# andrewkwolek/dynamic-visual-slam

Measured on AMD Instinct MI355X. Metric: frames/sec ORB+match @1280x720x2000kp, higher is better.
Workload: dtype u8

## Files before the change

### dynamic-visual-slam_amd/csrc/orb.hip

```cpp
#include <math.h>
#include <stdlib.h>
#include <string.h>
#include <algorithm>
#include <new>
#include <chrono>
#include <vector>
#include "common.h"
#include "cv_round.h"
#include "device_mem.h"
#ifdef DVS_TEST_HOOKS
#include "../../include/dvslam_hip_test.h"
#endif
#include "orb_kernels.h"

namespace dvs {

void launch_cand_mask(const Geom* d_geom, const Cell* d_cells, const CandMask& mk, uint32_t* cand, int* cellCount, int nimg, int c0, int c1,
                      hipStream_t st);

static inline short sat_short(int v) { return (short)(v < -32768 ? -32768 : (v > 32767 ? 32767 : v)); }
static inline uint64_t align_up(uint64_t v, uint64_t a) { return (v + a - 1) / a * a; }

}

// ... 43 lines not shown
  DeviceBuf<int> d_nodeof, d_celloff, d_candtotal;
  DeviceBuf<dvs_keypoint> d_kps;
  DeviceBuf<u8> d_desc;
  DeviceBuf<int> d_nout;
  PinnedBuf<dvs_keypoint> h_kps;
  PinnedBuf<u8> h_desc;
  PinnedBuf<int> h_nout;
  DeviceBuf<u8> d_mask;
  size_t octree_smem = 0;
  int octree_nmax = 0, octree_ptscap = 0;
  int oct_ncls = 0;
  int oct_l0[4] = {0, 0, 0, 0};
  size_t oct_smem_cls[3] = {0, 0, 0};
  int oct_nmax_cls[3] = {0, 0, 0}, oct_ptscap_cls[3] = {0, 0, 0};

  dvs_status ready(PyrSlot& s) { return s.pyr.get() ? DVS_OK : s.pyr.alloc(batch * geom.frameBytes + 256); }
  dvs_status ready(BlurSlot& s) { return s.blur.get() ? DVS_OK : s.blur.alloc(batch * geom.frameBytes); }
  dvs_status ready(CandSlot& s) {
    if (s.cellcount.get()) return DVS_OK;
    if (!s.done) DVS_HIP(s.done.create());
    DVS_TRY(s.cand.alloc(batch * geom.candPerFrame));
    return s.cellcount.alloc(batch * geom.totalCells);
  }
  dvs_status ready(LvlSlot& s) {
    if (s.lvlkp.get()) return DVS_OK;
    DVS_TRY(s.lvlcount.alloc(batch * geom.nlevels));
    return s.lvlkp.alloc(batch * (size_t)geom.kpBlock);
  }
  template <class Slot> dvs_status turn(Ring<Slot>& r) { r.advance(); return ready(r.cur()); }
  void rewind(int depth) { blur.rewind(depth); cand.rewind(depth); lvl.rewind(depth); pyr.depth = depth; }
};

enum {
  kEvFork,
  kEvBlur,
  kEvStart,
  kEvChainGate,
  kEvOct,
  kEvEnd,
  kEvPrefetch,
  kEvCount = kEvPrefetch + 2
};

struct dvs_orb {
  dvs_orb_params prm;
  int device = 0;
  hipStream_t own_stream = nullptr, stream = nullptr;
  hipStream_t pf_stream = nullptr;
  hipStream_t aux_stream = nullptr;
  Event ev[kEvCount];
  int pf_idx = 0;
  Event ev_level[DVS_MAX_LEVELS];
  bool overlap = true;
  bool single_stream = false;
  int max_batch = 1;
  std::vector<float> scale, inv_scale, sigma2, inv_sigma2;
  std::vector<int> feat_per_level;
  int umax[16];
  int rows = 0, cols = 0;
  Workspace ws;
  int ring = 3;
  int async_run = 0;
  Ring<Event> ev_outs;
  int out_gen = 0;
  bool out_pending = false;
  bool defer_outputs = false;
  hipEvent_t output_event = nullptr;
  hipEvent_t guard_event = nullptr;
  hipEvent_t after_fast_event = nullptr;
  hipEvent_t gate_event = nullptr;
  bool pf_joined = false;
  const u8* next_hint = nullptr;
  struct ChainGraph { const u8* img0; uint64_t step0, fstride0; int nimg; u8* pyr; hipGraph_t graph; hipGraphExec_t exec; };
  std::vector<ChainGraph> chain_graphs;
  int env_chain_graph = -1;
  int64_t chain_graph_launches = 0;
  bool pf_valid = false;
  const u8* pf_img = nullptr; uint64_t pf_step = 0, pf_fstride = 0; int pf_nimg = 0;
  int env_cascade = -1;
  int fast_byte_dma = 0;
  int env_blur_mfma = 0;
  int env_oct_threads = 0;
  int env_host_poll = 1;
  int env_desc_order = 1;
  PinnedBuf<int> h_seq;
  DeviceBuf<int> d_ticket;
  int export_seq = 0;
  bool async_oct = false, last_async = false;
  hipStream_t tail_stream = nullptr;
  CandMask mask{};
  int last_nimg = 0;
  ImgSrc last_src{};
  StageTimer timer;
};

namespace {

void drop_chain_graphs(dvs_orb* h) {
  for (auto& c : h->chain_graphs) {
    if (c.exec) (void)hipGraphExecDestroy(c.exec);
    if (c.graph) (void)hipGraphDestroy(c.graph);
  }
  h->chain_graphs.clear();
}

void free_workspace(dvs_orb* h) {
  h->ws = Workspace{};
  drop_chain_graphs(h);
  h->rows = h->cols = 0;
  h->out_gen = 0; h->pf_valid = false; h->next_hint = nullptr;
}

dvs_status quiesce(dvs_orb* h) {
  DVS_HIP(hipStreamSynchronize(h->stream));
  if (h->aux_stream) DVS_HIP(hipStreamSynchronize(h->aux_stream));
  if (h->pf_stream) DVS_HIP(hipStreamSynchronize(h->pf_stream));
  if (h->out_pending) DVS_HIP(hipEventSynchronize(h->ev_outs.cur()));
  h->out_pending = false;
  return DVS_OK;
}

void build_ctor_tables(dvs_orb* h) {
  const int nl = h->prm.nlevels;
  const double scaleFactor = (double)h->prm.scale_factor;
  h->scale.assign(nl, 0.f); h->sigma2.assign(nl, 0.f); h->inv_scale.assign(nl, 0.f); h->inv_sigma2.assign(nl, 0.f);
  h->scale[0] = 1.0f; h->sigma2[0] = 1.0f;
  for (int i = 1; i < nl; i++) {
    h->scale[i] = (float)(h->scale[i - 1] * scaleFactor);
    h->sigma2[i] = h->scale[i] * h->scale[i];
  }
  for (int i = 0; i < nl; i++) { h->inv_scale[i] = 1.0f / h->scale[i]; h->inv_sigma2[i] = 1.0f / h->sigma2[i]; }
  h->feat_per_level.assign(nl, 0);
  const float factor = (float)(1.0f / scaleFactor);
  float desired = h->prm.nfeatures * (1 - factor) / (1 - (float)pow((double)factor, (double)nl));
  int sum = 0;
  for (int l = 0; l < nl - 1; l++) {
    h->feat_per_level[l] = cv_round_f(desired);
    sum += h->feat_per_level[l];
    desired *= factor;
  }
  h->feat_per_level[nl - 1] = std::max(h->prm.nfeatures - sum, 0);
  int v, v0;
  const int vmax = cv_floor_f(kHalfPatch * sqrtf(2.f) / 2 + 1);
  const int vmin = cv_ceil_f(kHalfPatch * sqrtf(2.f) / 2);
  const double hp2 = kHalfPatch * kHalfPatch;
  for (v = 0; v <= vmax; ++v) h->umax[v] = cv_round_d(sqrt(hp2 - v * v));
  for (v = kHalfPatch, v0 = 0; v >= vmin; --v) {
    while (h->umax[v0] == h->umax[v0 + 1]) ++v0;
    h->umax[v] = v0;
    ++v0;
  }
}

void level_size(const dvs_orb* h, int rows, int cols, int level, int& lr, int& lc) {
  const float s = h->inv_scale[level];
  lc = cv_round_f((float)cols * s);
  lr = cv_round_f((float)rows * s);
}

void build_axis_table(int ssize, int dsize, bool clamp_like_x, std::vector<int>& ofs, std::vector<int>& coef) {
  const double inv_scale = (double)dsize / ssize;
  const double scale = 1. / inv_scale;
  for (int d = 0; d < dsize; d++) {
    float fx = (float)((d + 0.5) * scale - 0.5);
    int sx = cv_floor_f(fx);
    fx -= sx;
// ... 582 lines not shown

  if (h->overlap) {
    if (h->guard_event && !will_defer) { DVS_HIP(hipStreamWaitEvent(h->aux_stream, h->guard_event, 0)); h->guard_event = nullptr; }
    if (h->pf_valid && !sharded && !(h->defer_outputs && h->output_event)) { DVS_HIP(hipStreamWaitEvent(h->aux_stream, h->ev[kEvPrefetch + h->pf_idx], 0)); h->pf_joined = true; }
  }

  const bool tail = async && h->tail_stream != nullptr;
  if (tail) {
    h->timer.begin(DVS_STAGE_BLUR, st);
    launch_blur(h, src, nimg, st, cascade);
    h->timer.end(st);
  }

  if (ov) {
    int tail = G.nlevels;
    while (tail > 2 && G.lv[tail - 1].nCells * 16 < G.totalCells) tail--;
    for (int l = 0; l <= tail && l < G.nlevels; l++) {
      const int lastl = l == tail ? G.nlevels - 1 : l;
      if (lastl > 0) DVS_HIP(hipStreamWaitEvent(st, h->ev_level[lastl], 0));
      h->timer.begin(DVS_STAGE_FAST, st, l == 0);
      launch_fast(h, src, nimg, st, G.lv[l].cellBase, G.lv[lastl].cellBase + G.lv[lastl].nCells);
      h->timer.end(st);
    }
  } else {
    h->timer.begin(DVS_STAGE_FAST, st);
    if (sharded) {
      for (int l = 0; l < G.nlevels; l++)
        if ((src.levelMask >> l) & 1u) launch_fast(h, src, nimg, st, G.lv[l].cellBase, G.lv[l].cellBase + G.lv[l].nCells);
    } else {
      launch_fast(h, src, nimg, st, 0, G.totalCells);
    }
    h->timer.end(st);
  }
  hipStream_t bst = h->overlap ? h->aux_stream : st;
  hipEvent_t ev_fastdone = h->after_fast_event ? h->after_fast_event : h->ev[kEvFork];
  if (h->after_fast_event || h->overlap) DVS_HIP(hipEventRecord(ev_fastdone, st));

  if (pend) {
    DVS_TRY(W.turn(W.lvl));
  }
  hipStream_t qs = async ? bst : st;
  if (async) DVS_HIP(hipStreamWaitEvent(bst, ev_fastdone, 0));
  const int blurRows = (G.blurStrips + kOctTMax / 64 - 1) / (kOctTMax / 64);
  const bool fuse_blur = h->single_stream && !async && !sharded && !(h->env_blur_mfma && W.blur_mfma_ok) &&
                         blur_stream_ok(h, src, cascade) && (long)nimg * (G.nlevels + blurRows) <= 256;
  h->timer.begin(DVS_STAGE_OCTREE, qs);
  if (fuse_blur) {
    if (h->guard_event) { DVS_HIP(hipStreamWaitEvent(qs, h->guard_event, 0)); h->guard_event = nullptr; }
    hipLaunchKernelGGL(k_octree_blur, dim3(nimg, G.nlevels + blurRows), dim3(kOctTMax), W.octree_smem, qs, W.d_geom.get(), W.cand.cur().cand.get(), W.cand.cur().cellcount.get(),
                       W.d_celloff.get(), W.d_pts.get(), W.d_nodeof.get(), W.d_candtotal.get(), W.lvl.cur().lvlkp.get(), W.lvl.cur().lvlcount.get(), W.octree_nmax, W.octree_ptscap, src.levelMask,
                       G.nlevels, W.d_strips.get(), G.blurStrips, src, W.blur.cur().blur.get());
  } else {
    launch_octree(h, nimg, qs, src.levelMask, async && G.nlevels * nimg > 256);
  }
  h->timer.end(qs);
  if (async) { DVS_HIP(hipEventRecord(W.cand.cur().done, qs)); W.cand.cur().done_valid = true; }

  if (async) {}
  else if (bst != st) DVS_HIP(hipStreamWaitEvent(bst, ev_fastdone, 0));
  else if (h->guard_event) DVS_HIP(hipStreamWaitEvent(st, h->guard_event, 0));
  hipEvent_t late_guard = bst != st ? h->guard_event : nullptr;
  h->guard_event = nullptr;
  if (!tail && !fuse_blur) {
    h->timer.begin(DVS_STAGE_BLUR, bst);
    launch_blur(h, src, nimg, bst, cascade);
    h->timer.end(bst);
  }

  hipStream_t dst = st;
  if (will_defer) {
    dst = tail ? h->tail_stream : bst;
    if (tail) {
      DVS_HIP(hipStreamWaitEvent(dst, W.cand.cur().done, 0));
    } else if (!async) {
      DVS_HIP(hipEventRecord(h->ev[kEvOct], st));
      DVS_HIP(hipStreamWaitEvent(bst, h->ev[kEvOct], 0));
    }
    if (late_guard) DVS_HIP(hipStreamWaitEvent(dst, late_guard, 0));
  } else if (bst != st) {
    DVS_HIP(hipEventRecord(h->ev[kEvBlur], bst));
    DVS_HIP(hipStreamWaitEvent(st, h->ev[kEvBlur], 0));
  }
  h->timer.begin(DVS_STAGE_DESCRIBE, dst);
  if (h->env_desc_order && nimg >= 16) {
    hipLaunchKernelGGL(k_kp_order, dim3(nimg, G.nlevels), dim3(256), 0, dst, W.d_geom.get(), W.lvl.cur().lvlkp.get(), W.lvl.cur().lvlcount.get(), W.d_kpsorted.get(), W.d_kpsortidx.get());
    hipLaunchKernelGGL(k_describe, dim3((G.kpBlock + 4 * kDescKP - 1) / (4 * kDescKP), nimg), dim3(256), 0, dst, W.d_geom.get(), src, W.blur.cur().blur.get(),
                       W.d_kpsorted.get(), W.d_kpsortidx.get(), W.lvl.cur().lvlcount.get(), d_kps, d_desc, d_nout, capacity);
  } else {
    hipLaunchKernelGGL(k_describe, dim3((G.kpBlock + 4 * kDescKP - 1) / (4 * kDescKP), nimg), dim3(256), 0, dst, W.d_geom.get(), src, W.blur.cur().blur.get(),
                       W.lvl.cur().lvlkp.get(), W.d_kpident.get(), W.lvl.cur().lvlcount.get(), d_kps, d_desc, d_nout, capacity);
  }
  h->timer.end(dst);
  if (will_defer) {
    h->ev_outs.advance();
    h->out_gen++;
    DVS_HIP(hipEventRecord(h->ev_outs.cur(), dst));
    DVS_HIP(hipEventRecord(h->output_event, dst));
    h->out_pending = true;
    h->gate_event = nullptr;
  } else {
    h->gate_event = (may_defer && h->output_event) ? h->output_event : h->ev[kEvEnd];
    DVS_HIP(hipEventRecord(h->gate_event, st));
  }
  DVS_HIP(hipGetLastError());
  h->last_nimg = nimg;
  h->last_src = src;
  return DVS_OK;
}

}

extern "C" {

static dvs_status orb_create(const dvs_orb_params* params, int32_t device, bool single_stream, bool on_stream, hipStream_t ext, dvs_orb** out);
dvs_status dvs_orb_create(const dvs_orb_params* params, int32_t device, dvs_orb** out) { return orb_create(params, device, false, false, nullptr, out); }
DVS_HOOK dvs_status dvs_orb_create_single_stream(const dvs_orb_params* params, int32_t device, dvs_orb** out) { return orb_create(params, device, true, false, nullptr, out); }
DVS_HOOK dvs_status dvs_orb_create_on_stream(const dvs_orb_params* params, int32_t device, void* hip_stream, dvs_orb** out) {
  return orb_create(params, device, true, true, (hipStream_t)hip_stream, out);
}

static dvs_status orb_create(const dvs_orb_params* params, int32_t device, bool single_stream, bool on_stream, hipStream_t ext, dvs_orb** out) {
  DVS_ARG(params && out);
  *out = nullptr;
  DVS_ARG(params->nlevels >= 1 && params->nlevels <= DVS_MAX_LEVELS);
  DVS_ARG(params->nfeatures >= 0 && params->scale_factor > 1.0f && params->max_batch >= 0);
  DVS_TRY(check_device(device));
  dvs_orb* h = new (std::nothrow) dvs_orb();
  if (!h) { set_error("out of host memory"); return DVS_ERR_HIP; }
  h->prm = *params;
  bool allzero = true;
  for (int i = 0; i < 7; i++) allzero = allzero && params->gauss_kernel[i] == 0;
  if (allzero) { const int k[7] = {18, 34, 48, 56, 48, 34, 18}; memcpy(h->prm.gauss_kernel, k, sizeof(k)); }
  int ksum = 0;
  for (int i = 0; i < 7; i++) {
    ksum += h->prm.gauss_kernel[i];
    if (h->prm.gauss_kernel[i] < 0 || h->prm.gauss_kernel[i] > 255) ksum = 1 << 20;
  }
  if (ksum > 257) { delete h; set_error("gauss_kernel sum %d would overflow the Q8.8 row buffer", ksum); return DVS_ERR_ARG; }
  h->device = device;
  h->max_batch = params->max_batch > 0 ? params->max_batch : 1;
  if (on_stream) {
    h->stream = ext;
  } else {
    hipError_t e = hipStreamCreateWithFlags(&h->own_stream, hipStreamNonBlocking);
    if (e != hipSuccess) { delete h; set_error("hipStreamCreate: %s", hipGetErrorString(e)); return DVS_ERR_HIP; }
    h->stream = h->own_stream;
  }
  h->single_stream = single_stream;
  h->overlap = env_int("DVS_NO_OVERLAP", 0) == 0 && !single_stream;
  h->env_cascade = env_int("DVS_CASCADE", -1);
  h->env_chain_graph = env_int("DVS_CHAIN_GRAPH", -1);
  h->env_blur_mfma = env_int("DVS_BLUR_MFMA", 0);
  h->env_host_poll = env_int("DVS_HOST_POLL", 1);
  h->env_oct_threads = env_int("DVS_OCT_T", 0);
  h->env_desc_order = env_int("DVS_DESC_ORDER", 1);
  if (h->env_oct_threads != 0 && h->env_oct_threads != kOctT && h->env_oct_threads != kOctTMax) h->env_oct_threads = 0;
  h->fast_byte_dma = probe_byte_dma(device, h->stream) && env_int("DVS_FAST_BYTE_DMA", 1);
  int prio_lo = 0, prio_hi = 0;
  (void)hipDeviceGetStreamPriorityRange(&prio_lo, &prio_hi);
  bool ok = single_stream || (hipStreamCreateWithPriority(&h->aux_stream, hipStreamNonBlocking, prio_lo) == hipSuccess &&
                              hipStreamCreateWithPriority(&h->pf_stream, hipStreamNonBlocking, prio_hi) == hipSuccess);
  for (Event& e : h->ev) ok = ok && e.create() == hipSuccess;
  for (Event& e : h->ev_outs.slot) ok = ok && e.create() == hipSuccess;
  for (int l = 1; l < params->nlevels; l++) ok = ok && h->ev_level[l].create() == hipSuccess;
  h->ev_outs.rewind(h->ring - 1);
  if (!ok) {
    dvs_orb_destroy(h);
    set_error("stream / event creation failed");
    return DVS_ERR_HIP;
  }
  build_ctor_tables(h);
  *out = h;
  return DVS_OK;
}

void dvs_orb_destroy(dvs_orb* h) {
  if (!h) return;
  (void)hipSetDevice(h->device);
  (void)quiesce(h);
  h->timer.resolve();
  free_workspace(h);
  if (h->aux_stream) (void)hipStreamDestroy(h->aux_stream);
  if (h->pf_stream) (void)hipStreamDestroy(h->pf_stream);
  if (h->own_stream) (void)hipStreamDestroy(h->own_stream);
  delete h;
}

int32_t dvs_orb_max_keypoints(const dvs_orb* h) { return h ? h->prm.nfeatures + 3 * h->prm.nlevels : 0; }

dvs_status dvs_orb_set_stream(dvs_orb* h, void* s) {
  DVS_ARG(h);
  DVS_HIP(hipSetDevice(h->device));
  DVS_HIP(hipStreamSynchronize(h->stream));
  h->stream = (hipStream_t)s;
  return DVS_OK;
}
DVS_HOOK dvs_status dvs_orb_set_overlap(dvs_orb* h, int32_t on) {
  DVS_ARG(h);
  DVS_HIP(hipSetDevice(h->device));
  if (on && h->single_stream) { set_error("dvs_orb_set_overlap: this extractor was created with one stream only"); return DVS_ERR_UNSUPPORTED; }
  DVS_TRY(quiesce(h));
  h->pf_valid = false; h->pf_joined = false;
  h->overlap = on != 0;
  return DVS_OK;
}
DVS_HOOK dvs_status dvs_orb_set_async_quadtree(dvs_orb* h, int32_t on) {
  DVS_ARG(h);
  if (on && h->single_stream) { set_error("dvs_orb_set_async_quadtree: this extractor was created with one stream only"); return DVS_ERR_UNSUPPORTED; }
  DVS_HIP(hipSetDevice(h->device));
  DVS_TRY(quiesce(h));
  h->last_async = false;
  h->async_oct = on != 0;
  return DVS_OK;
}
DVS_HOOK int64_t dvs_orb_chain_graph_launches(const dvs_orb* h) { return h ? h->chain_graph_launches : 0; }

DVS_HOOK dvs_status dvs_orb_set_tail_stream(dvs_orb* h, void* hip_stream) {
  DVS_ARG(h);
  DVS_HIP(hipSetDevice(h->device));
  DVS_TRY(quiesce(h));
  h->tail_stream = (hipStream_t)hip_stream;
  h->ring = hip_stream ? 4 : 3;
  h->ws.rewind(h->ring); h->ev_outs.rewind(h->ring - 1); h->out_gen = 0; h->async_run = 0;
  for (CandSlot& c : h->ws.cand.slot) c.done_valid = false;
  h->last_async = false;
  return DVS_OK;
}
DVS_HOOK dvs_status dvs_orb_use_own_stream(dvs_orb* h) {
  DVS_ARG(h);
  if (!h->own_stream) { set_error("dvs_orb_use_own_stream: this extractor was created on a caller's stream and has none of its own"); return DVS_ERR_UNSUPPORTED; }
  DVS_HIP(hipSetDevice(h->device));
  DVS_HIP(hipStreamSynchronize(h->stream));
  h->stream = h->own_stream;
  return DVS_OK;
}
void* dvs_orb_get_stream(dvs_orb* h) { return h ? (void*)h->stream : nullptr; }

dvs_status dvs_orb_synchronize(dvs_orb* h) {
// ... 336 lines not shown
```

### dynamic-visual-slam_amd/csrc/orb_kernels.h

```cpp
#pragma once
#include <hip/hip_runtime.h>
#include "glibc_sincosf.h"
#include "lsort.h"
#include "orb_geom.h"
#include "orb_device_common.h"

namespace dvs {

typedef uint8_t u8;

struct ImgSrc {
  const u8* img0;
  uint64_t step0;
  uint64_t fstride0;
  u8* pyr;
  uint32_t levelMask;
  int32_t slotted;
};

__device__ __forceinline__ const u8* level_ptr(const Geom* g, const ImgSrc& s, int f, int l, int& pitch) {
  if (l == 0) { pitch = (int)s.step0; return s.img0 + (uint64_t)f * s.fstride0; }
  pitch = g->lv[l].pitch;
  return s.pyr + (uint64_t)f * g->frameBytes + g->lv[l].off;
}
// ... 1562 lines not shown
  if (!((src.levelMask >> it.level) & 1u)) return;
  const int lane = lane_id(), m = lane & 31, half = lane >> 5;
  const LevelGeom& L = g->lv[it.level];
  int pitch;
  const u8* img = level_ptr(g, src, f, it.level, pitch);
  u8* dst = blur + (uint64_t)f * g->frameBytes + L.off;
  const int W = L.w, H = L.h, dp = L.pitch;
  const int c0 = it.strip * 128 + 32 * wv;
  if (c0 >= W) return;
  const int ti = (it.tab + wv) * 2;
  const bv4i Bh1 = __builtin_bit_cast(bv4i, tab[(ti + 0) * 64 + lane]), Bh2 = __builtin_bit_cast(bv4i, tab[(ti + 1) * 64 + lane]);
  const bv4i Av0 = __builtin_bit_cast(bv4i, tab[(avt * 2 + 0) * 64 + lane]), Av1 = __builtin_bit_cast(bv4i, tab[(avt * 2 + 1) * 64 + lane]);
  const bv4i bias = {(int)0x80808080u, (int)0x80808080u, (int)0x80808080u, (int)0x80808080u};
  const bv16i zero = {0, 0, 0, 0, 0, 0, 0, 0, 0, 0, 0, 0, 0, 0, 0, 0};
  constexpr uint32_t kC = 65536u + (32768u << 8);
  const uint32_t col1 = (uint32_t)min(max(c0 - 16 + 16 * half, 0), pitch - 16), col2 = (uint32_t)min(max(c0 + 16 + 16 * half, 0), pitch - 16);
  auto row_off = [&](int vr) -> uint32_t {
    int r = vr < 0 ? -vr : vr;
    r = r >= H ? 2 * H - 2 - r : r;
    r = min(max(r, 0), H - 1);
    return (uint32_t)r * (uint32_t)pitch;
  };
  bv4i r1, r2;
  auto issue = [&](int b) {
    const uint32_t ro = row_off(32 * b - 3 + m);
    r1 = *reinterpret_cast<const bv4i*>(img + ro + col1);
    r2 = *reinterpret_cast<const bv4i*>(img + ro + col2);
  };
  auto hcomp = [&](const bv4i& x1, const bv4i& x2, bv4i& hi, bv4i& lo) {
    bv16i acc = __builtin_amdgcn_mfma_i32_32x32x32_i8(x1 ^ bias, Bh1, zero, 0, 0, 0);
    acc = __builtin_amdgcn_mfma_i32_32x32x32_i8(x2 ^ bias, Bh2, acc, 0, 0, 0);
    uint32_t P[8];
#pragma unroll
    for (int q = 0; q < 8; q++) P[q] = __builtin_amdgcn_perm((uint32_t)acc[2 * q + 1], (uint32_t)acc[2 * q], 0x05040100u);
#pragma unroll
    for (int d = 0; d < 4; d++) {
      hi[d] = (int)__builtin_amdgcn_perm(P[2 * d + 1], P[2 * d], 0x07050301u);
      lo[d] = (int)(__builtin_amdgcn_perm(P[2 * d + 1], P[2 * d], 0x06040200u) ^ 0x80808080u);
    }
  };
  const int ocol = c0 + 16 * half;
  uint32_t so = (uint32_t)(32 * it.t0 + m) * (uint32_t)dp + (uint32_t)ocol;
  auto vtile = [&](int t, const bv4i& chi, const bv4i& clo, const bv4i& nhi, const bv4i& nlo) {
    bv16i lo = __builtin_amdgcn_mfma_i32_32x32x32_i8(clo, Av0, zero, 0, 0, 0);
    lo = __builtin_amdgcn_mfma_i32_32x32x32_i8(nlo, Av1, lo, 0, 0, 0);
#pragma unroll
    for (int k = 0; k < 16; k++) lo[k] = (int)(((uint32_t)lo[k] + kC) >> 8);
    bv16i u = __builtin_amdgcn_mfma_i32_32x32x32_i8(chi, Av0, lo, 0, 0, 0);
    u = __builtin_amdgcn_mfma_i32_32x32x32_i8(nhi, Av1, u, 0, 0, 0);
    uint32_t o[4];
#pragma unroll
    for (int d = 0; d < 4; d++) {
      const uint32_t p01 = __builtin_amdgcn_perm((uint32_t)u[4 * d + 1], (uint32_t)u[4 * d], 0x0c0c0501u);
      const uint32_t p23 = __builtin_amdgcn_perm((uint32_t)u[4 * d + 3], (uint32_t)u[4 * d + 2], 0x0c0c0501u);
      o[d] = p01 | (p23 << 16);
    }
    const auto s02 = __builtin_amdgcn_permlane32_swap(o[0], o[2], false, false);
    const auto s13 = __builtin_amdgcn_permlane32_swap(o[1], o[3], false, false);
    if (32 * t + m < H && ocol < W) *reinterpret_cast<uint4*>(dst + so) = make_uint4(s02[0], s02[1], s13[0], s13[1]);
    so += 32u * (uint32_t)dp;
  };
  bv4i hiA, loA, hiB, loB;
  issue(it.t0);
  bv4i x1 = r1, x2 = r2;
  issue(it.t0 + 1);
  hcomp(x1, x2, hiA, loA);
  const int tend = it.t0 + it.nt;
  for (int t = it.t0; t < tend; t += 2) {
    x1 = r1; x2 = r2;
    if (t + 1 < tend) issue(t + 2);
    hcomp(x1, x2, hiB, loB);
    vtile(t, hiA, loA, hiB, loB);
    if (t + 1 < tend) {
      x1 = r1; x2 = r2;
      if (t + 2 < tend) issue(t + 3);
      hcomp(x1, x2, hiA, loA);
      vtile(t + 1, hiB, loB, hiA, loA);
    }
  }
}

constexpr int kDescKP = 8;
constexpr int kWinR = 18, kWinRows = 2 * kWinR + 1, kWinPitch = 48;
__global__ __launch_bounds__(256) void k_kp_order(const Geom* __restrict__ g, const uint32_t* __restrict__ lvlKp, const int* __restrict__ lvlKpCount,
                                                  uint32_t* __restrict__ sortedKp, uint32_t* __restrict__ sortedIdx) {
  __shared__ uint32_t key[kMaxQuota + 8];
  const int f = blockIdx.x, level = blockIdx.y;
  const LevelGeom& L = g->lv[level];
  const int n = min(lvlKpCount[f * g->nlevels + level], min(L.N + 4, kMaxQuota + 8));
  const uint32_t* in = lvlKp + (uint64_t)f * g->kpBlock + L.kpOff;
  uint32_t* outK = sortedKp + (uint64_t)f * g->kpBlock + L.kpOff;
  uint32_t* outI = sortedIdx + (uint64_t)f * g->kpBlock + L.kpOff;
  for (int i = threadIdx.x; i < n; i += 256) {
    const uint32_t pk = in[i];
    key[i] = ((uint32_t)(pt_y(pk) >> 5) << 20) | ((uint32_t)(pt_x(pk) >> 7) << 12) | (uint32_t)i;
  }
  __syncthreads();
  for (int i = threadIdx.x; i < n; i += 256) {
    const uint32_t k = key[i];
    int rank = 0;
    for (int j = 0; j < n; j++) rank += key[j] < k ? 1 : 0;
    outK[rank] = in[i];
    outI[rank] = (uint32_t)i;
  }
}

__global__ __launch_bounds__(256) void k_describe(const Geom* __restrict__ g, ImgSrc src, const u8* __restrict__ blur,
                                                  const uint32_t* __restrict__ lvlKp, const uint32_t* __restrict__ lvlKpIdx, const int* __restrict__ lvlKpCount,
                                                  dvs_keypoint* __restrict__ outKp, u8* __restrict__ outDesc,
                                                  int* __restrict__ nOut, int capacity) {
  typedef uint4 __attribute__((aligned(1))) uint4u;
  __shared__ __attribute__((aligned(16))) u8 win[4][2][kWinRows * kWinPitch];
  DVS_CHAIN_PRIO();
  const int wg = xcd_contiguous_id();
  const int f = wg / (int)gridDim.x, bx = wg - f * (int)gridDim.x;
  const int lane = lane_id();
  const int wv = __builtin_amdgcn_readfirstlane(threadIdx.x >> 6);
  const int nl = g->nlevels;
  const int* cnt = lvlKpCount + f * nl;
  const int slot0 = (bx * 4 + wv) * kDescKP;
  if (bx == 0 && threadIdx.x == 0) {
    if (src.slotted) {
      for (int l = 0; l < nl; l++) nOut[f * nl + l] = cnt[l];
    } else {
      int total = 0;
      for (int l = 0; l < nl; l++) total += cnt[l];
      nOut[f] = min(total, capacity);
    }
  }
  if (slot0 >= g->kpBlock) return;
  const int slot = min(slot0 + (lane & 7), g->kpBlock - 1);
  const uint32_t pkRaw = lvlKp[(uint64_t)f * g->kpBlock + slot];
  const uint32_t idxRaw = lvlKpIdx[(uint64_t)f * g->kpBlock + slot];
  int level = 0, pre = 0, acc = 0;
  for (int l = 0; l < nl; l++) {
    if (slot >= g->lv[l].kpOff) { level = l; pre = acc; }
    acc += cnt[l];
  }
  const LevelGeom& L = g->lv[level];
  const bool inlist = slot - L.kpOff < cnt[level];
  const int idx = inlist ? (int)idxRaw : slot - L.kpOff;
  const int gi = src.slotted ? L.kpOff + idx : pre + idx;
  const bool valid = slot0 + (lane & 7) < g->kpBlock && inlist && gi < capacity;
  if ((__ballot(valid) & 0xffull) == 0) return;
  const uint32_t pk = valid ? pkRaw : 0u;
  const int lvl = valid ? level : 0;
  const int x = pt_x(pk) + kMinBorder + (valid ? 0 : 3), y = pt_y(pk) + kMinBorder + (valid ? 0 : 3);
  const uint64_t pyrOff = (uint64_t)f * g->frameBytes + g->lv[lvl].off;
  const u8* imgL = lvl == 0 ? src.img0 + (uint64_t)f * src.fstride0 : src.pyr + pyrOff;
  const int pitchL = lvl == 0 ? (int)src.step0 : g->lv[lvl].pitch;
  const u8* blurL = blur + pyrOff;
  const int bpL = g->lv[lvl].pitch;
#define DVS_RL(v, i) __builtin_amdgcn_readlane((int)(v), (i))
#define DVS_RLP(p, i) reinterpret_cast<const u8*>(((uint64_t)(uint32_t)DVS_RL((uint32_t)((uint64_t)(p) >> 32), i) << 32) | (uint32_t)DVS_RL((uint32_t)(uint64_t)(p), i))
  const int prow = min(lane >> 1, 2 * kHalfPatch), half = lane & 1;
  const int v = prow - kHalfPatch;
  const int pcol = half ? 1 : -kHalfPatch;
  uint4 d[kDescKP];
#pragma unroll
  for (int i = 0; i < kDescKP; i++) {
    const u8* ib = DVS_RLP(imgL, i);
    const int pi = DVS_RL(pitchL, i), xi = DVS_RL(x, i), yi = DVS_RL(y, i);
    d[i] = *reinterpret_cast<const uint4u*>(ib + (uint32_t)(mul_i24(yi + v, pi) + xi + pcol));
  }
  const int e0 = lane, e1 = 64 + lane;
  const int wr0 = e0 / 3, wc0 = e0 - 3 * wr0, wr1 = min(e1 / 3, kWinRows - 1), wc1 = e1 - 3 * (e1 / 3);
  const bool w1ok = e1 < kWinRows * 3;
  static_assert(kDescKP == 8, "the window registers below are named per keypoint");
  uint4 wq0_0, wq0_1, wq0_2, wq0_3, wq0_4, wq0_5, wq0_6, wq0_7, wq1_0, wq1_1, wq1_2, wq1_3, wq1_4, wq1_5, wq1_6, wq1_7;
#define DVS_REQUEST_WINDOW(i)                                                                                  \
  {                                                                                                            \
    const u8* bb = DVS_RLP(blurL, i);                                                                          \
    const int bp = DVS_RL(bpL, i), xi = DVS_RL(x, i), yi = DVS_RL(y, i);                                       \
    const int xa = (xi - kWinR) & ~3;   \
    const u8* o = bb + (int64_t)(yi - kWinR) * bp + xa;                                                        \
    wq0_##i = *reinterpret_cast<const uint4*>(o + (uint32_t)(mul_i24(wr0, bp) + 16 * wc0));                    \
    wq1_##i = *reinterpret_cast<const uint4*>(o + (uint32_t)(mul_i24(wr1, bp) + 16 * wc1));                    \
  }
  DVS_REQUEST_WINDOW(0) DVS_REQUEST_WINDOW(1) DVS_REQUEST_WINDOW(2) DVS_REQUEST_WINDOW(3)
  float px0[4], py0[4], px1[4], py1[4];
#pragma unroll
  for (int r = 0; r < 4; r++) {
    const int pat = reinterpret_cast<const int*>(c_pattern)[64 * r + lane];
    px0[r] = (float)(int8_t)(pat & 0xff); py0[r] = (float)(int8_t)((pat >> 8) & 0xff);
    px1[r] = (float)(int8_t)((pat >> 16) & 0xff); py1[r] = (float)(int8_t)((pat >> 24) & 0xff);
  }
  const uint32_t* wt = g->icw[lane];
  const uint32_t w0 = wt[0], w1 = wt[1], w2 = wt[2], w3 = wt[3], w4 = wt[4], w5 = wt[5], w6 = wt[6], w7 = wt[7];
  int q[2 * kDescKP];
#pragma unroll
  for (int i = 0; i < kDescKP; i++) {
    uint32_t su = __builtin_amdgcn_udot4(d[i].x, w0, 0u, false);
    su = __builtin_amdgcn_udot4(d[i].y, w1, su, false);
    su = __builtin_amdgcn_udot4(d[i].z, w2, su, false);
    su = __builtin_amdgcn_udot4(d[i].w, w3, su, false);
    uint32_t sm = __builtin_amdgcn_udot4(d[i].x, w4, 0u, false);
    sm = __builtin_amdgcn_udot4(d[i].y, w5, sm, false);
    sm = __builtin_amdgcn_udot4(d[i].z, w6, sm, false);
    sm = __builtin_amdgcn_udot4(d[i].w, w7, sm, false);
    q[i] = (int)su - kHalfPatch * (int)sm;
    q[kDescKP + i] = v * (int)sm;
  }
  DVS_REQUEST_WINDOW(4) DVS_REQUEST_WINDOW(5) DVS_REQUEST_WINDOW(6) DVS_REQUEST_WINDOW(7)
#define DVS_BFLY(n, o)                                        \
  {                                                           \
    const bool hi = (lane & (o)) != 0;                        \
    _Pragma("unroll") for (int j = 0; j < (n); j++) {         \
      const int keep = hi ? q[(n) + j] : q[j];                \
      const int send = hi ? q[j] : q[(n) + j];                \
      q[j] = keep + __shfl_xor(send, (o));                    \
    }                                                         \
  }
  DVS_BFLY(8, 32) DVS_BFLY(4, 16) DVS_BFLY(2, 8) DVS_BFLY(1, 4)
#undef DVS_BFLY
  int tot = q[0];
  tot += __shfl_xor(tot, 2);
  tot += __shfl_xor(tot, 1);
  const int other = __shfl_xor(tot, 32);
  const int m10 = lane < 32 ? tot : other, m01 = lane < 32 ? other : tot;
  const float angleK = fast_atan2_deg((float)m01, (float)m10);
  const float factorPI = (float)(3.14159265358979323846 / 180.f);
  const float arad = __fmul_rn(angleK, factorPI);
  const float cosK = gsc::cosf_(arad), sinK = gsc::sinf_(arad);
  const unsigned vmask = (unsigned)(__ballot(valid) & 0xffull);
  constexpr int kCsLane = 4;
  const int giL = gi;
  auto brief = [&](const int i, const uint4& wa, const uint4& wb) __attribute__((always_inline)) {
    u8* wl = win[wv][i & 1];
    *reinterpret_cast<uint4*>(wl + wr0 * kWinPitch + 16 * wc0) = wa;
    if (w1ok) *reinterpret_cast<uint4*>(wl + wr1 * kWinPitch + 16 * wc1) = wb;
    const int xi = DVS_RL(x, i);
    const int wxi = xi - ((xi - kWinR) & ~3);
    wave_lds_fence();
    const float a = __builtin_bit_cast(float, DVS_RL(__builtin_bit_cast(int, cosK), kCsLane * i));
    const float b = __builtin_bit_cast(float, DVS_RL(__builtin_bit_cast(int, sinK), kCsLane * i));
    const int bco = kWinR * kWinPitch + wxi - 32 * kWinPitch - 0x4B000020;
    unsigned long long words[4];
    typedef float f32x2 __attribute__((ext_vector_type(2)));
    const f32x2 a2 = {a, a}, b2 = {b, b};
#pragma unroll
    for (int r = 0; r < 4; r++) {
      constexpr float kRound = 8388640.0f;
      const f32x2 kR2 = {kRound, kRound};
      const f32x2 pxv = {px0[r], px1[r]}, pyv = {py0[r], py1[r]};
      const f32x2 rowv = (pxv * b2 + pyv * a2) + kR2;
      const f32x2 colv = (pxv * a2 - pyv * b2) + kR2;
      const float fr0 = rowv[0], fr1 = rowv[1], fc0 = colv[0], fc1 = colv[1];
      const int r0 = __builtin_bit_cast(int, fr0), r1 = __builtin_bit_cast(int, fr1);
      const int c0 = __builtin_bit_cast(int, fc0), c1 = __builtin_bit_cast(int, fc1);
      const int t0 = wl[mad_i24(r0, kWinPitch, c0) + bco];
      const int t1 = wl[mad_i24(r1, kWinPitch, c1) + bco];
      words[r] = __ballot(t0 < t1);
    }
    if ((vmask >> i) & 1u) {
      const int gii = DVS_RL(giL, i);
      if (lane < 4) {
        const unsigned long long w = lane == 0 ? words[0] : lane == 1 ? words[1] : lane == 2 ? words[2] : words[3];
        reinterpret_cast<unsigned long long*>(outDesc + ((uint64_t)f * capacity + gii) * 32)[lane] = w;
      }
    }
  };
  brief(0, wq0_0, wq1_0); brief(1, wq0_1, wq1_1); brief(2, wq0_2, wq1_2); brief(3, wq0_3, wq1_3);
  brief(4, wq0_4, wq1_4); brief(5, wq0_5, wq1_5); brief(6, wq0_6, wq1_6); brief(7, wq0_7, wq1_7);
  const float angle = __shfl(angleK, kCsLane * (lane & 7));
  if (lane < kDescKP && valid) {
    dvs_keypoint kp;
    kp.x = (float)x; kp.y = (float)y;
    if (level != 0) { kp.x = __fmul_rn(kp.x, L.scale); kp.y = __fmul_rn(kp.y, L.scale); }
    kp.size = L.kpSize;
    kp.angle = angle;
    kp.response = (float)pt_s(pk);
    kp.octave = level;
    kp.class_id = -1;
    outKp[(uint64_t)f * capacity + gi] = kp;
  }
#undef DVS_REQUEST_WINDOW
#undef DVS_RL
#undef DVS_RLP
}

struct LevelBlockLayout { uint64_t blockBytes, kpsOff, descOff; int nl, kpBlock; int kpOff[DVS_MAX_LEVELS]; int owner[DVS_MAX_LEVELS]; };

__global__ __launch_bounds__(256) void k_merge_levels(LevelBlockLayout Y, const u8* __restrict__ blocks, int nimg, dvs_keypoint* __restrict__ outKp,
                                                      u8* __restrict__ outDesc, int capacity, int* __restrict__ nOut) {
  const int f = blockIdx.y;
  const int slot = blockIdx.x * 256 + threadIdx.x;
  int level = 0, pre = 0, acc = 0, cntL = 0;
  for (int l = 0; l < Y.nl; l++) {
    const int c = reinterpret_cast<const int*>(blocks + (uint64_t)Y.owner[l] * Y.blockBytes)[f * Y.nl + l];
    if (slot >= Y.kpOff[l]) { level = l; pre = acc; cntL = c; }
    acc += c;
  }
  if (slot == 0) nOut[f] = min(acc, capacity);
  if (slot >= Y.kpBlock) return;
  const int idx = slot - Y.kpOff[level], gi = pre + idx;
  if (idx >= cntL || gi >= capacity) return;
  const u8* blk = blocks + (uint64_t)Y.owner[level] * Y.blockBytes;
  const uint32_t* sk = reinterpret_cast<const uint32_t*>(blk + Y.kpsOff) + ((uint64_t)f * Y.kpBlock + slot) * 7;
  uint32_t* dk = reinterpret_cast<uint32_t*>(outKp) + ((uint64_t)f * capacity + gi) * 7;
#pragma unroll
  for (int k = 0; k < 7; k++) dk[k] = sk[k];
  const uint4* sd = reinterpret_cast<const uint4*>(blk + Y.descOff) + ((uint64_t)f * Y.kpBlock + slot) * 2;
  uint4* dd = reinterpret_cast<uint4*>(outDesc) + ((uint64_t)f * capacity + gi) * 2;
  dd[0] = sd[0]; dd[1] = sd[1];
}


__global__ __launch_bounds__(256) void k_export_host(int nimg, int cap, const uint32_t* __restrict__ kps, const uint32_t* __restrict__ desc,
                                                     const int* __restrict__ nout, uint32_t* __restrict__ hkps, uint32_t* __restrict__ hdesc,
                                                     int* __restrict__ hnout, int* __restrict__ ticket, int* __restrict__ hseq, int seq) {
  const int f = blockIdx.y;
  const int n = min(nout[f], cap);
  const uint32_t* ks = kps + (uint64_t)f * cap * 7;
  const uint32_t* ds = desc + (uint64_t)f * cap * 8;
  uint32_t* kd = hkps + (uint64_t)f * cap * 7;
  uint32_t* dd = hdesc + (uint64_t)f * cap * 8;
  for (int i = blockIdx.x * 256 + threadIdx.x; i < n * 7; i += gridDim.x * 256) kd[i] = ks[i];
  for (int i = blockIdx.x * 256 + threadIdx.x; i < n * 8; i += gridDim.x * 256) dd[i] = ds[i];
  if (blockIdx.x == 0 && threadIdx.x == 0) hnout[f] = nout[f];
  __threadfence_system();
  __syncthreads();
  if (threadIdx.x == 0) {
    const int total = gridDim.x * gridDim.y;
    if (atomicAdd(ticket, 1) == total - 1) {
      *ticket = 0;
      __threadfence_system();
      *reinterpret_cast<volatile int*>(hseq) = seq;
      __threadfence_system();
    }
  }
// ... 4 lines not shown
```

### dynamic-visual-slam_amd/csrc/util.hip

```cpp
#include <stdlib.h>
#include <string.h>
#include "common.h"
#ifdef DVS_TEST_HOOKS
#include "../../include/dvslam_hip_test.h"
#endif

extern "C" char** environ;

namespace dvs {

static thread_local char g_err[1024] = "";

void set_error(const char* fmt, ...) {
  va_list ap;
  va_start(ap, fmt);
  vsnprintf(g_err, sizeof(g_err), fmt, ap);
  va_end(ap);
}

namespace {
struct EnvSwitch { const char* name; int allowed[4]; int nallowed; };
const EnvSwitch kSwitches[] = {
    {"DVS_NO_OVERLAP", {0, 1}, 2},
    {"DVS_CASCADE", {-1, 0, 1}, 3},
    {"DVS_CHAIN_GRAPH", {-1, 0, 1}, 3},
    {"DVS_BLUR_MFMA", {0, 1, 2}, 3},
    {"DVS_HOST_POLL", {0, 1}, 2},
    {"DVS_OCT_T", {0, 256, 512}, 3},
    {"DVS_DESC_ORDER", {0, 1}, 2},
    {"DVS_FAST_BYTE_DMA", {0, 1}, 2},
    {"DVS_MATCH_MFMA", {0, 1}, 2},
    {"DVS_MATCH_LDS", {0, 1}, 2},
    {"DVS_LM_POLL", {0, 1}, 2},
    {"DVS_LM_SPECULATE", {0, 1}, 2},
};
const EnvSwitch* find_switch(const char* name, size_t len) {
  for (const EnvSwitch& s : kSwitches)
    if (strlen(s.name) == len && strncmp(s.name, name, len) == 0) return &s;
  return nullptr;
}
}

dvs_status env_check() {
  for (char** e = environ; e && *e; e++) {
    if (strncmp(*e, "DVS_", 4) != 0) continue;
    const char* eq = strchr(*e, '=');
    if (!eq) continue;
    const EnvSwitch* s = find_switch(*e, (size_t)(eq - *e));
    if (!s) {
      set_error("unknown environment switch %.*s (the library reads: DVS_NO_OVERLAP DVS_CASCADE DVS_CHAIN_GRAPH DVS_BLUR_MFMA DVS_HOST_POLL DVS_OCT_T "
                "DVS_DESC_ORDER DVS_FAST_BYTE_DMA DVS_MATCH_MFMA DVS_MATCH_LDS DVS_LM_POLL DVS_LM_SPECULATE)", (int)(eq - *e), *e);
      return DVS_ERR_ARG;
    }
    char* end = nullptr;
    const long v = strtol(eq + 1, &end, 10);
    bool ok = end != eq + 1 && *end == 0;
    if (ok) { ok = false; for (int i = 0; i < s->nallowed; i++) ok = ok || s->allowed[i] == (int)v; }
    if (!ok) {
      char list[64] = ""; size_t o = 0;
      for (int i = 0; i < s->nallowed; i++) o += (size_t)snprintf(list + o, sizeof(list) - o, "%s%d", i ? ", " : "", s->allowed[i]);
      set_error("%s=%s: not a value of this switch (allowed: %s)", s->name, eq + 1, list);
      return DVS_ERR_ARG;
    }
  }
  return DVS_OK;
}

int env_switch(const char* name, int dflt) {
  const char* v = getenv(name);
  return v && find_switch(name, strlen(name)) ? atoi(v) : dflt;
}

dvs_status check_device(int device) {
  DVS_TRY(env_check());
  int n = 0;
  hipError_t e = hipGetDeviceCount(&n);
  if (e != hipSuccess || n <= 0) {
    set_error("no HIP device visible (%s); libdvslam_hip has no CPU fallback", e == hipSuccess ? "count 0" : hipGetErrorString(e));
    (void)hipGetLastError();
    return DVS_ERR_NO_DEVICE;
  }
  if (device < 0 || device >= n) { set_error("device %d out of range (0..%d)", device, n - 1); return DVS_ERR_ARG; }
  DVS_HIP(hipSetDevice(device));
  return DVS_OK;
}

void StageTimer::begin(int stage, hipStream_t s, bool count_call) {
  if (!on) return;
  if (npending >= kMaxPending) resolve();
  Pending& p = pending[npending];
  if (npool < 2 * (npending + 1)) {
    hipEventCreate(&pool[npool++]);
    hipEventCreate(&pool[npool++]);
  }
  p.a = pool[2 * npending]; p.b = pool[2 * npending + 1]; p.stage = stage; p.count = count_call;
  hipEventRecord(p.a, s);
  cur = npending++;
}
void StageTimer::end(hipStream_t s) {
  if (!on || cur < 0) return;
  hipEventRecord(pending[cur].b, s);
  cur = -1;
}
void StageTimer::resolve() {
  for (int i = 0; i < npending; i++) {
    hipEventSynchronize(pending[i].b);
    float t = 0;
    if (hipEventElapsedTime(&t, pending[i].a, pending[i].b) == hipSuccess) { ms[pending[i].stage] += t; if (pending[i].count) calls[pending[i].stage]++; }
  }
  npending = 0;
}
void StageTimer::reset() { resolve(); memset(ms, 0, sizeof(ms)); memset(calls, 0, sizeof(calls)); }
StageTimer::~StageTimer() { for (int i = 0; i < npool; i++) hipEventDestroy(pool[i]); }

}

#ifdef DVS_TEST_HOOKS
__global__ void k_test_spin(unsigned long long ticks) {
  const unsigned long long t0 = wall_clock64();
  while (wall_clock64() - t0 < ticks) __builtin_amdgcn_s_sleep(32);
}
#endif

extern "C" {

const char* dvs_last_error(void) { return dvs::g_err; }

int32_t dvs_device_count(void) {
  int n = 0;
  if (hipGetDeviceCount(&n) != hipSuccess) { (void)hipGetLastError(); return 0; }
  return n;
}

dvs_status dvs_stream_create(int32_t device, int32_t high_priority, void** out_stream) {
// ... 125 lines not shown
```

Before: 147,200.

## Add steer table option, DPP butterflies and vectorized rank count in describe

Adds an opt-in (DVS_DESC_TABLE) templated describe path that precomputes per-keypoint rotated coordinate products in LDS and looks them up per pattern point instead of multiplying. Always-on changes replace the later shuffle butterfly stages with DPP and permlane32 swaps, drop the w1ok guard on the second window store, and vectorize the rank-counting loop in k_kp_order with uint4 LDS reads and padding. Together these aim to cut cross-lane shuffle latency and LDS instruction count, but they rely on the padded window and key buffers being large enough.

New measurement: 147,300, median of 2. Within noise of the previous version (+0.1%).

```diff
diff --git a/dynamic-visual-slam_amd/csrc/orb.hip b/dynamic-visual-slam_amd/csrc/orb.hip
--- a/dynamic-visual-slam_amd/csrc/orb.hip
+++ b/dynamic-visual-slam_amd/csrc/orb.hip
@@ -149,6 +149,7 @@
   int env_blur_mfma = 0;
   int env_oct_threads = 0;
   int env_host_poll = 1;
+  int env_desc_table = 0;
   int env_desc_order = 1;
   PinnedBuf<int> h_seq;
   DeviceBuf<int> d_ticket;
@@ -897,12 +898,13 @@
     DVS_HIP(hipStreamWaitEvent(st, h->ev[kEvBlur], 0));
   }
   h->timer.begin(DVS_STAGE_DESCRIBE, dst);
+  const auto describe = h->env_desc_table ? k_describe<true> : k_describe<false>;
   if (h->env_desc_order && nimg >= 16) {
     hipLaunchKernelGGL(k_kp_order, dim3(nimg, G.nlevels), dim3(256), 0, dst, W.d_geom.get(), W.lvl.cur().lvlkp.get(), W.lvl.cur().lvlcount.get(), W.d_kpsorted.get(), W.d_kpsortidx.get());
-    hipLaunchKernelGGL(k_describe, dim3((G.kpBlock + 4 * kDescKP - 1) / (4 * kDescKP), nimg), dim3(256), 0, dst, W.d_geom.get(), src, W.blur.cur().blur.get(),
+    hipLaunchKernelGGL(describe, dim3((G.kpBlock + 4 * kDescKP - 1) / (4 * kDescKP), nimg), dim3(256), 0, dst, W.d_geom.get(), src, W.blur.cur().blur.get(),
                        W.d_kpsorted.get(), W.d_kpsortidx.get(), W.lvl.cur().lvlcount.get(), d_kps, d_desc, d_nout, capacity);
   } else {
-    hipLaunchKernelGGL(k_describe, dim3((G.kpBlock + 4 * kDescKP - 1) / (4 * kDescKP), nimg), dim3(256), 0, dst, W.d_geom.get(), src, W.blur.cur().blur.get(),
+    hipLaunchKernelGGL(describe, dim3((G.kpBlock + 4 * kDescKP - 1) / (4 * kDescKP), nimg), dim3(256), 0, dst, W.d_geom.get(), src, W.blur.cur().blur.get(),
                        W.lvl.cur().lvlkp.get(), W.d_kpident.get(), W.lvl.cur().lvlcount.get(), d_kps, d_desc, d_nout, capacity);
   }
   h->timer.end(dst);
@@ -969,6 +971,7 @@
   h->env_host_poll = env_int("DVS_HOST_POLL", 1);
   h->env_oct_threads = env_int("DVS_OCT_T", 0);
   h->env_desc_order = env_int("DVS_DESC_ORDER", 1);
+  h->env_desc_table = env_int("DVS_DESC_TABLE", 0);
   if (h->env_oct_threads != 0 && h->env_oct_threads != kOctT && h->env_oct_threads != kOctTMax) h->env_oct_threads = 0;
   h->fast_byte_dma = probe_byte_dma(device, h->stream) && env_int("DVS_FAST_BYTE_DMA", 1);
   int prio_lo = 0, prio_hi = 0;
diff --git a/dynamic-visual-slam_amd/csrc/orb_kernels.h b/dynamic-visual-slam_amd/csrc/orb_kernels.h
--- a/dynamic-visual-slam_amd/csrc/orb_kernels.h
+++ b/dynamic-visual-slam_amd/csrc/orb_kernels.h
@@ -1668,9 +1668,11 @@
 
 constexpr int kDescKP = 8;
 constexpr int kWinR = 18, kWinRows = 2 * kWinR + 1, kWinPitch = 48;
+constexpr int kSteerC = 13, kSteerN = 2 * kSteerC + 1;
 __global__ __launch_bounds__(256) void k_kp_order(const Geom* __restrict__ g, const uint32_t* __restrict__ lvlKp, const int* __restrict__ lvlKpCount,
                                                   uint32_t* __restrict__ sortedKp, uint32_t* __restrict__ sortedIdx) {
-  __shared__ uint32_t key[kMaxQuota + 8];
+  constexpr int kKeyCap = (kMaxQuota + 8 + 3) & ~3;
+  __shared__ __attribute__((aligned(16))) uint32_t key[kKeyCap];
   const int f = blockIdx.x, level = blockIdx.y;
   const LevelGeom& L = g->lv[level];
   const int n = min(lvlKpCount[f * g->nlevels + level], min(L.N + 4, kMaxQuota + 8));
@@ -1681,22 +1683,31 @@
     const uint32_t pk = in[i];
     key[i] = ((uint32_t)(pt_y(pk) >> 5) << 20) | ((uint32_t)(pt_x(pk) >> 7) << 12) | (uint32_t)i;
   }
+  const int n4 = (n + 3) & ~3;
+  if ((int)threadIdx.x < n4 - n) key[n + threadIdx.x] = 0xFFFFFFFFu;
   __syncthreads();
   for (int i = threadIdx.x; i < n; i += 256) {
     const uint32_t k = key[i];
     int rank = 0;
-    for (int j = 0; j < n; j++) rank += key[j] < k ? 1 : 0;
+    for (int j = 0; j < n4; j += 4) {
+      const uint4 kj = *reinterpret_cast<const uint4*>(key + j);
+      rank += (kj.x < k ? 1 : 0) + (kj.y < k ? 1 : 0) + (kj.z < k ? 1 : 0) + (kj.w < k ? 1 : 0);
+    }
     outK[rank] = in[i];
     outI[rank] = (uint32_t)i;
   }
 }
 
+template <bool kTable>
 __global__ __launch_bounds__(256) void k_describe(const Geom* __restrict__ g, ImgSrc src, const u8* __restrict__ blur,
                                                   const uint32_t* __restrict__ lvlKp, const uint32_t* __restrict__ lvlKpIdx, const int* __restrict__ lvlKpCount,
                                                   dvs_keypoint* __restrict__ outKp, u8* __restrict__ outDesc,
                                                   int* __restrict__ nOut, int capacity) {
+#pragma clang fp contract(off)
   typedef uint4 __attribute__((aligned(1))) uint4u;
+  typedef float f32x2 __attribute__((ext_vector_type(2)));
   __shared__ __attribute__((aligned(16))) u8 win[4][2][kWinRows * kWinPitch];
+  __shared__ f32x2 steer[kTable ? 4 : 1][2][kTable ? kSteerN : 1];
   DVS_CHAIN_PRIO();
   const int wg = xcd_contiguous_id();
   const int f = wg / (int)gridDim.x, bx = wg - f * (int)gridDim.x;
@@ -1751,7 +1762,6 @@
   }
   const int e0 = lane, e1 = 64 + lane;
   const int wr0 = e0 / 3, wc0 = e0 - 3 * wr0, wr1 = min(e1 / 3, kWinRows - 1), wc1 = e1 - 3 * (e1 / 3);
-  const bool w1ok = e1 < kWinRows * 3;
   static_assert(kDescKP == 8, "the window registers below are named per keypoint");
   uint4 wq0_0, wq0_1, wq0_2, wq0_3, wq0_4, wq0_5, wq0_6, wq0_7, wq1_0, wq1_1, wq1_2, wq1_3, wq1_4, wq1_5, wq1_6, wq1_7;
 #define DVS_REQUEST_WINDOW(i)                                                                                  \
@@ -1765,12 +1775,17 @@
   }
   DVS_REQUEST_WINDOW(0) DVS_REQUEST_WINDOW(1) DVS_REQUEST_WINDOW(2) DVS_REQUEST_WINDOW(3)
   float px0[4], py0[4], px1[4], py1[4];
+  int ox0[4], oy0[4], ox1[4], oy1[4];
 #pragma unroll
   for (int r = 0; r < 4; r++) {
     const int pat = reinterpret_cast<const int*>(c_pattern)[64 * r + lane];
     px0[r] = (float)(int8_t)(pat & 0xff); py0[r] = (float)(int8_t)((pat >> 8) & 0xff);
     px1[r] = (float)(int8_t)((pat >> 16) & 0xff); py1[r] = (float)(int8_t)((pat >> 24) & 0xff);
-  }
+    ox0[r] = ((int)(int8_t)(pat & 0xff) + kSteerC) * 8; oy0[r] = ((int)(int8_t)((pat >> 8) & 0xff) + kSteerC) * 8;
+    ox1[r] = ((int)(int8_t)((pat >> 16) & 0xff) + kSteerC) * 8; oy1[r] = ((int)(int8_t)((pat >> 24) & 0xff) + kSteerC) * 8;
+  }
+  const int tslot = min(lane, kSteerN - 1);
+  const float tcoord = (float)(tslot - kSteerC);
   const uint32_t* wt = g->icw[lane];
   const uint32_t w0 = wt[0], w1 = wt[1], w2 = wt[2], w3 = wt[3], w4 = wt[4], w5 = wt[5], w6 = wt[6], w7 = wt[7];
   int q[2 * kDescKP];
@@ -1797,13 +1812,22 @@
       q[j] = keep + __shfl_xor(send, (o));                    \
     }                                                         \
   }
-  DVS_BFLY(8, 32) DVS_BFLY(4, 16) DVS_BFLY(2, 8) DVS_BFLY(1, 4)
+#define DVS_BFLY_DPP(n, shl, shr, lo, hi)                                                   \
+  _Pragma("unroll") for (int j = 0; j < (n); j++) {                                          \
+    const int a_ = __builtin_amdgcn_update_dpp(q[j], q[(n) + j], (shr), 0xf, (hi), false);   \
+    const int b_ = __builtin_amdgcn_update_dpp(q[(n) + j], q[j], (shl), 0xf, (lo), false);   \
+    q[j] = a_ + b_;                                                                          \
+  }
+  DVS_BFLY(8, 32) DVS_BFLY(4, 16)
+  DVS_BFLY_DPP(2, 0x108, 0x118, 0x3, 0xc)
+  DVS_BFLY_DPP(1, 0x104, 0x114, 0x5, 0xa)
 #undef DVS_BFLY
+#undef DVS_BFLY_DPP
   int tot = q[0];
-  tot += __shfl_xor(tot, 2);
-  tot += __shfl_xor(tot, 1);
-  const int other = __shfl_xor(tot, 32);
-  const int m10 = lane < 32 ? tot : other, m01 = lane < 32 ? other : tot;
+  tot += __builtin_amdgcn_update_dpp(0, tot, 0x4e, 0xf, 0xf, false);
+  tot += __builtin_amdgcn_update_dpp(0, tot, 0xb1, 0xf, 0xf, false);
+  const auto mm = __builtin_amdgcn_permlane32_swap((unsigned)tot, (unsigned)tot, false, false);
+  const int m10 = (int)mm[0], m01 = (int)mm[1];
   const float angleK = fast_atan2_deg((float)m01, (float)m10);
   const float factorPI = (float)(3.14159265358979323846 / 180.f);
   const float arad = __fmul_rn(angleK, factorPI);
@@ -1811,27 +1835,49 @@
   const unsigned vmask = (unsigned)(__ballot(valid) & 0xffull);
   constexpr int kCsLane = 4;
   const int giL = gi;
+  auto steer_sum = [](const f32x2 X, const f32x2 Y) __attribute__((always_inline)) {
+    f32x2 r;
+    asm("v_pk_add_f32 %0, %1, %2 op_sel:[1,0] op_sel_hi:[0,1] neg_hi:[0,1]" : "=v"(r) : "v"(X), "v"(Y));
+    return r;
+  };
   auto brief = [&](const int i, const uint4& wa, const uint4& wb) __attribute__((always_inline)) {
+#pragma clang fp contract(off)
     u8* wl = win[wv][i & 1];
     *reinterpret_cast<uint4*>(wl + wr0 * kWinPitch + 16 * wc0) = wa;
-    if (w1ok) *reinterpret_cast<uint4*>(wl + wr1 * kWinPitch + 16 * wc1) = wb;
+    *reinterpret_cast<uint4*>(wl + wr1 * kWinPitch + 16 * wc1) = wb;
     const int xi = DVS_RL(x, i);
     const int wxi = xi - ((xi - kWinR) & ~3);
-    wave_lds_fence();
     const float a = __builtin_bit_cast(float, DVS_RL(__builtin_bit_cast(int, cosK), kCsLane * i));
     const float b = __builtin_bit_cast(float, DVS_RL(__builtin_bit_cast(int, sinK), kCsLane * i));
+    const u8* tb = reinterpret_cast<const u8*>(steer[kTable ? wv : 0][i & 1]);
+    if constexpr (kTable) steer[wv][i & 1][tslot] = f32x2{tcoord * a, tcoord * b};
+    wave_lds_fence();
+    f32x2 X0[4], Y0[4], X1[4], Y1[4];
+    if constexpr (kTable) {
+#pragma unroll
+      for (int r = 0; r < 4; r++) {
+        X0[r] = *reinterpret_cast<const f32x2*>(tb + ox0[r]); Y0[r] = *reinterpret_cast<const f32x2*>(tb + oy0[r]);
+        X1[r] = *reinterpret_cast<const f32x2*>(tb + ox1[r]); Y1[r] = *reinterpret_cast<const f32x2*>(tb + oy1[r]);
+      }
+    }
+    const f32x2 a2 = {a, a}, b2 = {b, b};
     const int bco = kWinR * kWinPitch + wxi - 32 * kWinPitch - 0x4B000020;
     unsigned long long words[4];
-    typedef float f32x2 __attribute__((ext_vector_type(2)));
-    const f32x2 a2 = {a, a}, b2 = {b, b};
 #pragma unroll
     for (int r = 0; r < 4; r++) {
       constexpr float kRound = 8388640.0f;
       const f32x2 kR2 = {kRound, kRound};
-      const f32x2 pxv = {px0[r], px1[r]}, pyv = {py0[r], py1[r]};
-      const f32x2 rowv = (pxv * b2 + pyv * a2) + kR2;
-      const f32x2 colv = (pxv * a2 - pyv * b2) + kR2;
-      const float fr0 = rowv[0], fr1 = rowv[1], fc0 = colv[0], fc1 = colv[1];
+      float fr0, fc0, fr1, fc1;
+      if constexpr (kTable) {
+        const f32x2 rc0 = steer_sum(X0[r], Y0[r]) + kR2;
+        const f32x2 rc1 = steer_sum(X1[r], Y1[r]) + kR2;
+        fr0 = rc0[0]; fc0 = rc0[1]; fr1 = rc1[0]; fc1 = rc1[1];
+      } else {
+        const f32x2 pxv = {px0[r], px1[r]}, pyv = {py0[r], py1[r]};
+        const f32x2 rowv = (pxv * b2 + pyv * a2) + kR2;
+        const f32x2 colv = (pxv * a2 - pyv * b2) + kR2;
+        fr0 = rowv[0]; fr1 = rowv[1]; fc0 = colv[0]; fc1 = colv[1];
+      }
       const int r0 = __builtin_bit_cast(int, fr0), r1 = __builtin_bit_cast(int, fr1);
       const int c0 = __builtin_bit_cast(int, fc0), c1 = __builtin_bit_cast(int, fc1);
       const int t0 = wl[mad_i24(r0, kWinPitch, c0) + bco];
diff --git a/dynamic-visual-slam_amd/csrc/util.hip b/dynamic-visual-slam_amd/csrc/util.hip
--- a/dynamic-visual-slam_amd/csrc/util.hip
+++ b/dynamic-visual-slam_amd/csrc/util.hip
@@ -28,6 +28,7 @@
     {"DVS_HOST_POLL", {0, 1}, 2},
     {"DVS_OCT_T", {0, 256, 512}, 3},
     {"DVS_DESC_ORDER", {0, 1}, 2},
+    {"DVS_DESC_TABLE", {0, 1}, 2},
     {"DVS_FAST_BYTE_DMA", {0, 1}, 2},
     {"DVS_MATCH_MFMA", {0, 1}, 2},
     {"DVS_MATCH_LDS", {0, 1}, 2},
@@ -49,7 +50,7 @@
     const EnvSwitch* s = find_switch(*e, (size_t)(eq - *e));
     if (!s) {
       set_error("unknown environment switch %.*s (the library reads: DVS_NO_OVERLAP DVS_CASCADE DVS_CHAIN_GRAPH DVS_BLUR_MFMA DVS_HOST_POLL DVS_OCT_T "
-                "DVS_DESC_ORDER DVS_FAST_BYTE_DMA DVS_MATCH_MFMA DVS_MATCH_LDS DVS_LM_POLL DVS_LM_SPECULATE)", (int)(eq - *e), *e);
+                "DVS_DESC_ORDER DVS_DESC_TABLE DVS_FAST_BYTE_DMA DVS_MATCH_MFMA DVS_MATCH_LDS DVS_LM_POLL DVS_LM_SPECULATE)", (int)(eq - *e), *e);
       return DVS_ERR_ARG;
     }
     char* end = nullptr;
```
